# fractalclockwork/CS267_HW3

Hardware: NVIDIA B200
Metric: kmers_per_s_insert_plus_traverse (higher is better)
Workload: dtype u128

## Files before the change

### cs267_hw3_b200/csrc/capi.cu

```cuda
#include <algorithm>
#include <cmath>
#include <cstdio>
#include <cstdlib>
#include <cstring>
#include <string>
#include <vector>

#include <cub/device/device_radix_sort.cuh>

#include "../../include/kh_capi.h"
#include "kernels.cuh"
#include "ctable.cuh"

using namespace kh;

namespace {

struct DevBuf {
    void* p = nullptr;
    size_t cap = 0;
};

enum { EV_INS0, EV_INS1, EV_AS0, EV_WALK, EV_RANK, EV_AS1, EV_PACK0, EV_PACK1, EV_CLR0, EV_CLR1, EV_STAGE1, EV_BUILD0, EV_BUILD1, EV_COUNT };

// ... 1 lines not shown

struct kh_table {
    int k = 0, W = 1, device = 0, pl = 0, pb = 0, slot_bytes = 8, per_bucket = 4;
    int mlen = 0;
    int olen = 0;
    double lf = 0.5;
    u64 n_expected = 0, nbuckets = 0;
    cudaStream_t stream = nullptr, own_stream = nullptr, copy_stream = nullptr;
    void* table = nullptr;
    size_t table_bytes = 0;
    DevBuf starts;
    u64 n_starts = 0;
    DevBuf mask, tile_counts, tile_offs, scan_blocks;
    DevBuf part_cursor, grouped;
    DevBuf fine, chunk_cursor, overflow;
    int build_mode = 1;
    bool table_dirty = false;
    bool chunk_attr_set = false;
    int debug_cap_pct = 100;
    int partition_mode = -1;
    u64 part_bytes = 16ull << 20;
    bool part_attr_set = false;
    int ins_mode = 1;
    int warm_ahead = 1;
    Counters* d_ctr = nullptr;
    Counters* h_ctr = nullptr;
    DevBuf link, seglen, tmp, contig_len, contig_pre, contig_off, out;
    DevBuf stage[2], text_stage, scratch_a, scratch_b, scratch_c;
    DevBuf sort_keys[2], sort_vals[2], sort_tmp;
    void* h_out = nullptr; size_t h_out_cap = 0;
    void* h_off = nullptr; size_t h_off_cap = 0;
    u32 split_shift = 5, seg_chars = 64;
    cudaEvent_t ev[EV_COUNT] = {};
    cudaEvent_t ev_copied[2] = {}, ev_consumed[2] = {};
    cudaEvent_t ev_built = nullptr, ev_gathered = nullptr;
    bool have_ins = false, have_as = false, have_pack = false, have_clr = false, have_build = false, have_stage = false;
    u64 n_launches = 0;
    kh_stats stats = {};
    std::string err;
    int sm_count = 148, walk_blocks_per_sm = 0, rank_blocks_per_sm = 0;
    u64 last_contig_bytes = 0, last_n_contigs = 0;
    struct CtState {
        bool on = false, sealed = false, sharded = false, attr_set = false, connected = false;
        bool assembled = false;
        CtGeom g = {};
        CtCaps caps = {};
        CtPeers pe = {};
        u32 epoch = 0;
        u64 n_local_max = 0, n_total = 0, n_starts_max = 0, out_cap = 0;
        u64 n_starts_host = 0;
        DevBuf xin_vals, xin_chunk, xin_cnt, xin_done, xout_cursor, extra_vals, extra_chunk, extra_cnt, fine, chunk_cursor,
               chunk_base, pool_off, seg_base, ext_key, meta, pool, inbox, inbox_cnt, out_cursor, flags,
               answers, req_seg, g_link, g_meta, g_pool, g_hdr;
        bool slow = false;
        void* ipc_opened[kMaxRanks][24] = {};
    } ct;
    int ct_env = 1;
};

namespace {

int fail(kh_table* t, int status, const std::string& msg) {
    if (t) t->err = msg;
    return status;
}

#define KH_CUDA(t, expr)                                                                         \
    do {                                                                                         \
        cudaError_t e_ = (expr);                                                                 \
        if (e_ != cudaSuccess)                                                                   \
            return fail((t), e_ == cudaErrorMemoryAllocation ? KH_ERR_NOMEM : KH_ERR_CUDA,       \
                        std::string(#expr) + ": " + cudaGetErrorString(e_));                     \
    } while (0)

#define KH_TRY(expr)                  \
    do {                              \
        const int rc_ = (expr);       \
        if (rc_ != KH_OK) return rc_; \
    } while (0)

int ensure(kh_table* t, DevBuf& b, size_t bytes, bool keep = false) {
    if (bytes <= b.cap && b.p) return KH_OK;
    const size_t want = std::max<size_t>(256, bytes + bytes / 8);
    void* np = nullptr;
    KH_CUDA(t, cudaMalloc(&np, want));
    if (b.p) {
        if (keep && b.cap) KH_CUDA(t, cudaMemcpyAsync(np, b.p, b.cap, cudaMemcpyDeviceToDevice, t->stream));
        KH_CUDA(t, cudaStreamSynchronize(t->stream));
        KH_CUDA(t, cudaFree(b.p));
    }
    b.p = np;
    b.cap = want;
    return KH_OK;
}

int ensure_pinned(kh_table* t, void*& p, size_t& cap, size_t bytes) {
    if (bytes <= cap && p) return KH_OK;
    if (p) KH_CUDA(t, cudaFreeHost(p));
    p = nullptr; cap = 0;
    const size_t want = std::max<size_t>(4096, bytes + bytes / 8);
    KH_CUDA(t, cudaHostAlloc(&p, want, cudaHostAllocDefault));
    cap = want;
    return KH_OK;
}

int status_from_errors(kh_table* t, u32 e) {
// ... 378 lines not shown
    c.n_local_max = n_local_max; c.n_total = n_total; c.n_starts_max = n_starts_max; c.sharded = sharded;
    const u64 nb_alloc = (u64)((long double)n_exp / (long double)t->lf / per_bucket) + C + 64;
    if (!t->table || t->table_bytes < nb_alloc * 32) {
        if (t->table) { KH_CUDA(t, cudaStreamSynchronize(t->stream)); KH_CUDA(t, cudaFree(t->table)); t->table = nullptr; }
        KH_CUDA(t, cudaMalloc(&t->table, nb_alloc * 32));
        t->table_bytes = nb_alloc * 32;
    }
    t->nbuckets = nb_alloc;
    c.caps.nbuckets_alloc = nb_alloc;
    const double share = (double)std::max<u64>(n_local_max, 1) / (double)world;
    u64 xin_cap = world > 1 ? (u64)((share * 1.05 + 64.0 * std::sqrt(share + 1.0) + 4096.0) * t->debug_cap_pct / 100.0) : 8;
    xin_cap = std::max<u64>(8, (xin_cap + 7) & ~7ull);
    if (xin_cap >= 0xFFFFFFF0ull) return fail(t, KH_ERR_ARG, "receive buffer too large");
    c.caps.xin_cap = (u32)xin_cap;
    c.caps.extra_cap = (u32)std::min<u64>(0x7FFFFFF0ull, t->debug_cap_pct < 100 ? n_local_max * (u64)world + 65536 : n_exp / 16 + 65536);
    const u64 hcap = sharded ? std::min<u64>(std::max<u64>(n_starts_max, 1), n_local_max + 1) : 0;
    c.caps.hcap = (u32)hcap;
    const u64 seg_cap = hcap + n_exp + 64;
    if (seg_cap >= (u64)kLocalMask - 16 && sharded) return fail(t, KH_ERR_ARG, "too many segments per GPU for 28-bit local ids");
    c.caps.seg_cap = (u32)std::min<u64>(seg_cap, 0xFFFFFF00ull);
    c.caps.pool_cap = n_exp + 16 * C + 64;
    c.caps.inbox_cap = world > 1 ? (u32)std::min<u64>(0x7FFFFFF0ull, ((n_exp + n_local_max) / world) * 9 / 8 + 4096) : 1;
    c.out_cap = n_total + std::max<u64>(n_starts_max, 1) * (u64)(t->k + 1) + 64;
    KH_TRY(ensure(t, c.xin_vals, (u64)world * xin_cap * sizeof(V)));
    KH_TRY(ensure(t, c.xin_chunk, (u64)world * xin_cap * sizeof(u32)));
    KH_TRY(ensure(t, c.xin_cnt, kMaxRanks * sizeof(u32)));
    KH_TRY(ensure(t, c.xin_done, (kMaxRanks + 1) * sizeof(u32)));
    KH_TRY(ensure(t, c.xout_cursor, kMaxRanks * sizeof(u32)));
    KH_TRY(ensure(t, c.extra_vals, (u64)c.caps.extra_cap * sizeof(V)));
    KH_TRY(ensure(t, c.extra_chunk, (u64)c.caps.extra_cap * sizeof(u32)));
    KH_TRY(ensure(t, c.extra_cnt, 16));
    KH_TRY(ensure(t, c.fine, C * (u64)((slots_max + 15) & ~15u) * sizeof(V)));
    KH_TRY(ensure(t, c.chunk_cursor, (C + 1) * sizeof(u32)));
    KH_TRY(ensure(t, c.chunk_base, (C + 2) * sizeof(u32)));
    KH_TRY(ensure(t, c.pool_off, (C + 2) * sizeof(u32)));
    KH_TRY(ensure(t, c.seg_base, (C + 1) * sizeof(u32)));
    KH_TRY(ensure(t, c.pool, c.caps.pool_cap + 64));
    KH_TRY(ensure(t, c.inbox, (u64)world * c.caps.inbox_cap * sizeof(CtReq<W>)));
    KH_TRY(ensure(t, c.inbox_cnt, kMaxRanks * sizeof(u32)));
    KH_TRY(ensure(t, c.out_cursor, kMaxRanks * sizeof(u32)));
    KH_TRY(ensure(t, c.flags, 2 * kMaxRanks * sizeof(u32)));
    c.caps.g_seg_stride = world > 1 ? ((n_local_max + 1 + n_exp + 64 + 15) & ~15ull) : 0;
    c.caps.g_pool_stride = world > 1 ? ((c.caps.pool_cap + 64 + 15) & ~15ull) : 0;
    KH_TRY(ensure(t, c.answers, std::max<u64>(16, (u64)(world > 1 ? world : 0) * c.caps.inbox_cap * sizeof(u32))));
    KH_TRY(ensure(t, c.req_seg, std::max<u64>(16, (u64)(world > 1 ? world : 0) * c.caps.inbox_cap * sizeof(u32))));
    KH_TRY(ensure(t, c.g_link, std::max<u64>(16, (u64)world * c.caps.g_seg_stride * sizeof(u64))));
    KH_TRY(ensure(t, c.g_meta, std::max<u64>(16, (u64)world * c.caps.g_seg_stride * sizeof(u64))));
    KH_TRY(ensure(t, c.g_pool, std::max<u64>(16, (u64)world * c.caps.g_pool_stride)));
    KH_TRY(ensure(t, c.g_hdr, 2 * kMaxRanks * sizeof(u32)));
    if (sharded) {
        KH_TRY(ensure(t, t->link, seg_cap * sizeof(u64)));
        KH_TRY(ensure(t, c.meta, seg_cap * sizeof(u64)));
        KH_TRY(ensure(t, c.ext_key, seg_cap * sizeof(V)));
        KH_TRY(ensure(t, t->contig_len, (hcap + 2) * sizeof(u32)));
        KH_TRY(ensure(t, t->contig_pre, (hcap + 2) * sizeof(u32)));
        KH_TRY(ensure(t, t->contig_off, (hcap + 2) * sizeof(u64)));
        KH_TRY(ensure(t, t->out, c.out_cap));
        KH_TRY(ensure(t, t->starts, (hcap + 1) * sizeof(V)));
        const u64 ntiles = (n_local_max + kInsTile - 1) / kInsTile + 1;
        KH_TRY(ensure(t, t->mask, (ntiles + 1) * (kInsTile / 32) * sizeof(u32)));
        KH_TRY(ensure(t, t->tile_counts, (ntiles + 1) * sizeof(u32)));
        KH_TRY(ensure(t, t->tile_offs, (ntiles + 1) * sizeof(u64)));
        KH_TRY(ensure(t, t->scan_blocks, ((std::max(ntiles, hcap + 2) + kScanTile - 1) / kScanTile + 2) * sizeof(u64)));
    }
    KH_TRY(ct_reset_staging(t));
    KH_CUDA(t, cudaMemsetAsync(c.inbox_cnt.p, 0, kMaxRanks * sizeof(u32), t->stream));
    KH_CUDA(t, cudaMemsetAsync(c.flags.p, 0, 2 * kMaxRanks * sizeof(u32), t->stream));
    KH_CUDA(t, cudaStreamSynchronize(t->stream));
    if (!c.attr_set) {
        KH_CUDA(t, cudaFuncSetAttribute(ct_build_kernel<W>, cudaFuncAttributeMaxDynamicSharedMemorySize, (int)CtBuild<W>::kSmem));
        KH_CUDA(t, cudaFuncSetAttribute(ct_build_kernel<W>, cudaFuncAttributePreferredSharedMemoryCarveout, (int)cudaSharedmemCarveoutMaxShared));
        KH_CUDA(t, cudaFuncSetAttribute(ct_stage_kernel<W>, cudaFuncAttributeMaxDynamicSharedMemorySize, (int)ct_stage_smem(W, 8)));
        c.attr_set = true;
    }
    memset(&c.pe, 0, sizeof(c.pe));
    c.pe.world = world; c.pe.rank = rank;
    c.epoch = 0;
    ct_set_self(t);
    c.on = true; c.sealed = false;
    return KH_OK;
}

int ct_barrier(kh_table* t, int round = -1) {
    auto& c = t->ct;
    if (c.pe.world <= 1) return KH_OK;
    ++c.epoch;
    ct_barrier_kernel<<<1, 32, 0, t->stream>>>(c.pe, c.epoch & 0x7FFFFFFFu, t->d_ctr, round);
    ++t->n_launches;
    KH_CUDA(t, cudaGetLastError());
    return KH_OK;
}

template <int W>
int ct_stage(kh_table* t, const unsigned char* recs, u64 n) {
    typedef typename Slot<W>::value_t V;
    auto& c = t->ct;
    if (n == 0) return KH_OK;
    if (n >= 0xFFF00000ull) return fail(t, KH_ERR_ARG, "at most 2^32-2^20 records per insert call; split the batch");
    const u64 ntiles = (n + kInsTile - 1) / kInsTile;
    if (!c.sharded) {
        KH_TRY(ensure(t, t->mask, (ntiles + 1) * (kInsTile / 32) * sizeof(u32)));
        KH_TRY(ensure(t, t->tile_counts, (ntiles + 1) * sizeof(u32)));
        KH_TRY(ensure(t, t->tile_offs, (ntiles + 1) * sizeof(u64)));
        KH_TRY(ensure(t, t->scan_blocks, ((ntiles + kScanTile - 1) / kScanTile + 2) * sizeof(u64)));
        KH_TRY(ensure(t, t->starts, (c.n_starts_host + n + 1) * sizeof(V), true));
        c.caps.hcap = (u32)std::min<u64>(0xFFFFFF00ull, c.n_starts_host + n + 1);
// ... 7 lines not shown
    KH_TRY(device_scan(t, static_cast<u32*>(t->tile_counts.p), ntiles, static_cast<u64*>(t->tile_offs.p), &t->d_ctr->scan_total));
    ct_scatter_starts_kernel<W><<<(unsigned)((ntiles * 32 + 255) / 256), 256, 0, t->stream>>>(
        recs, n, t->k, static_cast<u32*>(t->mask.p), static_cast<u64*>(t->tile_offs.p), ntiles, static_cast<V*>(t->starts.p),
        t->d_ctr, c.caps.hcap);
    ct_bump_starts_kernel<<<1, 1, 0, t->stream>>>(t->d_ctr, c.caps.hcap);
    KH_CUDA(t, cudaGetLastError());
    t->n_launches += 3;
    KH_CUDA(t, cudaEventRecord(t->ev[EV_STAGE1], t->stream));
    t->have_stage = true;
    c.sealed = false; c.assembled = false;
    t->table_dirty = true;
    return KH_OK;
}

__global__ void ct_init_seal_kernel(Counters* c, u32 hcap) {
    c->next_seg = hcap;
    c->n_inserted = 0;
    c->n_duplicates = 0;
}
__global__ void ct_init_assemble_kernel(Counters* c) {
    c->n_nodes = 0;
    c->contig_bytes = 0;
    c->rank_rounds = 0;
    c->rank_done = 0;
    c->need_jump = 0;
    c->use_jump = 0;
    for (int i = 0; i < 40; ++i) c->flags[i] = 0;
}
__global__ void ct_reset_nodes_kernel(Counters* c) { c->n_nodes = 0; }

template <int W>
int ct_seal_publish(kh_table* t) {
    auto& c = t->ct;
    if (c.pe.world > 1) {
        ct_publish_xin_kernel<<<1, 32, 0, t->stream>>>(c.pe, c.caps, static_cast<const u32*>(c.xout_cursor.p));
        ++t->n_launches;
        KH_CUDA(t, cudaGetLastError());
    }
    return ct_barrier(t);
}
template <int W>
int ct_seal_build(kh_table* t) {
    typedef typename Slot<W>::value_t V;
    auto& c = t->ct;
    const u32 C = c.g.chunks_per_rank;
    if (!c.sharded) {
        const u64 hcap = c.n_starts_host + 1;
        const u64 seg_cap = hcap + std::max<u64>(t->n_expected, 1) + 64;
        if (seg_cap >= 0xFFFFFF00ull) return fail(t, KH_ERR_ARG, "too many segments for 32-bit ids");
        c.caps.hcap = (u32)hcap; c.caps.seg_cap = (u32)seg_cap;
        KH_TRY(ensure(t, t->link, seg_cap * sizeof(u64)));
        KH_TRY(ensure(t, c.meta, seg_cap * sizeof(u64)));
        KH_TRY(ensure(t, c.ext_key, seg_cap * sizeof(V)));
        ct_set_self(t);
    }
    ct_init_seal_kernel<<<1, 1, 0, t->stream>>>(t->d_ctr, c.caps.hcap);
    if (c.pe.world > 1) {
        u32* done = static_cast<u32*>(c.xin_done.p);
        ct_xin_scatter_kernel<W><<<(unsigned)t->sm_count * 8, 256, 0, t->stream>>>(
            static_cast<const V*>(c.xin_vals.p), static_cast<const u32*>(c.xin_chunk.p), static_cast<const u32*>(c.xin_cnt.p), done,
            c.g, c.caps, static_cast<u32*>(c.chunk_cursor.p), static_cast<V*>(c.fine.p), t->d_ctr);
        ct_extra_kernel<W><<<64, 256, 0, t->stream>>>(static_cast<const V*>(c.extra_vals.p), static_cast<const u32*>(c.extra_chunk.p),
                                                      static_cast<const u32*>(c.extra_cnt.p), done + kMaxRanks, c.caps, C,
                                                      static_cast<u32*>(c.chunk_cursor.p), static_cast<V*>(c.fine.p), t->d_ctr);
        ct_mark_filed_kernel<<<1, 32, 0, t->stream>>>(static_cast<const u32*>(c.xin_cnt.p), done, static_cast<const u32*>(c.extra_cnt.p),
                                                      done + kMaxRanks, c.caps, c.pe.world);
        t->n_launches += 3;
    }
    ct_layout_kernel<<<1, 1024, 0, t->stream>>>(static_cast<const u32*>(c.chunk_cursor.p), C, c.g, c.caps, (u32)Slot<W>::kPerBucket,
                                                CtBuild<W>::kMaxSlots, static_cast<u32*>(c.chunk_base.p), static_cast<u32*>(c.pool_off.p), t->d_ctr);
    t->n_launches += 2;
    KH_CUDA(t, cudaEventRecord(t->ev[EV_BUILD0], t->stream));
    ct_build_kernel<W><<<C, kCtBuildThreads, CtBuild<W>::kSmem, t->stream>>>(
        static_cast<const V*>(c.fine.p), static_cast<const u32*>(c.chunk_cursor.p), static_cast<const u32*>(c.chunk_base.p),
        static_cast<const u32*>(c.pool_off.p), static_cast<V*>(t->table), static_cast<u32*>(c.seg_base.p),
        static_cast<u64*>(t->link.p), static_cast<u64*>(c.meta.p), static_cast<V*>(c.ext_key.p),
        static_cast<unsigned char*>(c.pool.p), c.g, c.caps, t->d_ctr);
    KH_CUDA(t, cudaGetLastError());
    KH_CUDA(t, cudaEventRecord(t->ev[EV_BUILD1], t->stream));
    t->have_build = true;
    c.sealed = true;
    return KH_OK;
}

constexpr int kCtMaxRounds = 24;
constexpr int kCtParts = 8 + kCtMaxRounds;
constexpr u32 kCtWalkMaxSteps = 512;

template <int W>
int ct_assemble_part(kh_table* t, int part) {
    typedef typename Slot<W>::value_t V;
    auto& c = t->ct;
    const unsigned gb = (unsigned)t->sm_count * 8;
    u64* link = static_cast<u64*>(t->link.p);
    CtGathered gt = {};
    for (int r = 0; r < c.pe.world; ++r) {
        const bool me = r == c.pe.rank;
        gt.link[r] = me ? link : static_cast<const u64*>(c.g_link.p) + (u64)r * c.caps.g_seg_stride;
        gt.meta[r] = me ? static_cast<const u64*>(c.meta.p) : static_cast<const u64*>(c.g_meta.p) + (u64)r * c.caps.g_seg_stride;
        gt.pool[r] = me ? static_cast<const unsigned char*>(c.pool.p) : static_cast<const unsigned char*>(c.g_pool.p) + (u64)r * c.caps.g_pool_stride;
    }
    switch (part) {
    case 0:
        if (c.assembled) { c.sealed = false; c.assembled = false; }
        c.slow = false;
        KH_CUDA(t, cudaEventRecord(t->ev[EV_AS0], t->stream));
// ... 1 lines not shown
        return ct_barrier(t);
    case 1: {
        if (!c.sealed) { KH_TRY(ct_seal_build<W>(t)); KH_CUDA(t, cudaEventRecord(t->ev[EV_INS1], t->stream)); t->have_ins = true; }
        if (!c.sharded) {
            const u64 hc = c.n_starts_host;
            KH_TRY(ensure(t, t->contig_len, (hc + 3) * sizeof(u32)));
            KH_TRY(ensure(t, t->contig_pre, (hc + 3) * sizeof(u32)));
            KH_TRY(ensure(t, t->contig_off, (hc + 3) * sizeof(u64)));
            c.out_cap = t->h_ctr->n_inserted + c.n_starts_host * (u64)(t->k + 1) + 64;
            ct_set_self(t);
        }
        if (c.pe.world > 1) {
            KH_CUDA(t, cudaEventRecord(t->ev_built, t->stream));
            KH_CUDA(t, cudaStreamWaitEvent(t->copy_stream, t->ev_built, 0));
            ct_gather_kernel<<<gb, 256, 0, t->copy_stream>>>(c.pe, c.caps, link, static_cast<const u64*>(c.meta.p), static_cast<const unsigned char*>(c.pool.p),
                                                             static_cast<const u32*>(c.pool_off.p), c.g.chunks_per_rank, t->d_ctr, 0);
            KH_CUDA(t, cudaEventRecord(t->ev_gathered, t->copy_stream));
            ++t->n_launches;
        }
        ct_init_assemble_kernel<<<1, 1, 0, t->stream>>>(t->d_ctr);
        KH_CUDA(t, cudaMemsetAsync(c.out_cursor.p, 0, kMaxRanks * sizeof(u32), t->stream));
        ct_stub_kernel<W><<<std::max(1u, std::min(gb, (c.caps.hcap + 255u) / 256u)), 256, 0, t->stream>>>(
            static_cast<const V*>(t->starts.p), t->d_ctr, c.caps.hcap, link, static_cast<u64*>(c.meta.p), static_cast<V*>(c.ext_key.p));
        ct_resolve_kernel<W><<<gb, 256, 0, t->stream>>>(static_cast<const V*>(t->table), static_cast<const u32*>(c.chunk_base.p),
                                                        static_cast<const u32*>(c.seg_base.p), link, static_cast<const V*>(c.ext_key.p),
                                                        c.g, c.pe, c.caps, static_cast<u32*>(c.out_cursor.p), static_cast<u32*>(c.req_seg.p), t->d_ctr);
        if (c.pe.world > 1) { ct_publish_inbox_kernel<<<1, 32, 0, t->stream>>>(c.pe, c.caps, static_cast<const u32*>(c.out_cursor.p)); ++t->n_launches; }
        t->n_launches += 3;
        KH_CUDA(t, cudaGetLastError());
        return ct_barrier(t);
    }
    case 2:
        if (c.pe.world > 1) {
            ct_answer_kernel<W><<<gb, 256, 0, t->stream>>>(static_cast<const V*>(t->table), static_cast<const u32*>(c.chunk_base.p),
                                                           static_cast<const u32*>(c.seg_base.p), static_cast<const CtReq<W>*>(c.inbox.p),
                                                           static_cast<const u32*>(c.inbox_cnt.p), c.g, c.pe, c.caps);
            KH_CUDA(t, cudaGetLastError());
            ++t->n_launches;
        }
        return ct_barrier(t);
    case 3:
        if (c.pe.world > 1) {
            ct_apply_kernel<<<gb, 256, 0, t->stream>>>(link, static_cast<const u32*>(c.answers.p), static_cast<const u32*>(c.req_seg.p),
                                                       static_cast<const u32*>(c.out_cursor.p), c.caps, c.pe.world, c.pe.rank);
            ct_gather_kernel<<<gb, 256, 0, t->stream>>>(c.pe, c.caps, link, static_cast<const u64*>(c.meta.p), static_cast<const unsigned char*>(c.pool.p),
                                                        static_cast<const u32*>(c.pool_off.p), c.g.chunks_per_rank, t->d_ctr, 1);
            KH_CUDA(t, cudaStreamWaitEvent(t->stream, t->ev_gathered, 0));
            KH_CUDA(t, cudaGetLastError());
            t->n_launches += 2;
        }
        KH_CUDA(t, cudaEventRecord(t->ev[EV_WALK], t->stream));
        return ct_barrier(t);
    case 4:
        ct_walk_len_kernel<<<gb, 256, 0, t->stream>>>(gt, link, c.caps, t->k, kCtWalkMaxSteps, static_cast<u32*>(t->contig_len.p), t->d_ctr);
        KH_CUDA(t, cudaGetLastError());
        ++t->n_launches;
        return ct_barrier(t, -2);
    case 5: {
        KH_TRY(device_scan(t, static_cast<u32*>(t->contig_len.p), (u64)c.caps.hcap + 1, static_cast<u64*>(t->contig_off.p), &t->d_ctr->contig_bytes));
        KH_CUDA(t, cudaEventRecord(t->ev[EV_RANK], t->stream));
        ct_walk_emit_kernel<W><<<gb, 256, 0, t->stream>>>(gt, link, static_cast<const V*>(t->starts.p), c.caps, t->k, static_cast<const u32*>(t->contig_len.p),
                                                          static_cast<const u64*>(t->contig_off.p), c.out_cap, static_cast<char*>(t->out.p), t->d_ctr);
        KH_CUDA(t, cudaGetLastError());
        ++t->n_launches;
        KH_CUDA(t, cudaEventRecord(t->ev[EV_AS1], t->stream));
        t->have_as = true;
        return KH_OK;
    }
    case 6: {
        KH_TRY(read_counters(t));
        c.slow = (c.pe.world > 1 ? t->h_ctr->use_jump : t->h_ctr->need_jump) != 0;
        if (!c.slow) return KH_OK;
        c.assembled = true;
        ct_rank_round_kernel<<<gb, 256, 0, t->stream>>>(c.pe, link, c.caps, t->d_ctr, t->d_ctr->flags, 0);
        KH_CUDA(t, cudaGetLastError());
        ++t->n_launches;
        return ct_barrier(t, 0);
    }
    case 6 + kCtMaxRounds: {
        if (!c.slow) return KH_OK;
        ct_reset_nodes_kernel<<<1, 1, 0, t->stream>>>(t->d_ctr);
        ct_lengths_kernel<<<gb, 256, 0, t->stream>>>(c.pe, link, c.caps, t->k, static_cast<u32*>(t->contig_len.p),
                                                     static_cast<u32*>(t->contig_pre.p), t->d_ctr);
        ct_claim_kernel<<<gb, 256, 0, t->stream>>>(c.pe, link, c.caps, static_cast<const u32*>(t->contig_len.p), t->d_ctr);
        KH_CUDA(t, cudaGetLastError());
        t->n_launches += 3;
        KH_TRY(device_scan(t, static_cast<u32*>(t->contig_len.p), (u64)c.caps.hcap + 1, static_cast<u64*>(t->contig_off.p), &t->d_ctr->contig_bytes));
        KH_CUDA(t, cudaEventRecord(t->ev[EV_RANK], t->stream));
        return ct_barrier(t);
    }
    case 7 + kCtMaxRounds:
        if (!c.slow) return KH_OK;
        ct_emit_kernel<<<gb, 256, 0, t->stream>>>(c.pe, link, static_cast<const u64*>(c.meta.p), static_cast<const unsigned char*>(c.pool.p),
                                                  c.caps, t->d_ctr, t->k);
        ct_emit_heads_kernel<W><<<gb, 256, 0, t->stream>>>(static_cast<const V*>(t->starts.p), c.caps, t->k, static_cast<const u32*>(t->contig_len.p),
                                                          static_cast<const u64*>(t->contig_off.p), t->d_ctr, c.out_cap, static_cast<char*>(t->out.p));
        KH_CUDA(t, cudaGetLastError());
        t->n_launches += 2;
        KH_CUDA(t, cudaEventRecord(t->ev[EV_AS1], t->stream));
        t->have_as = true;
        return ct_barrier(t);
    default: {
        if (part < 7 || part >= 6 + kCtMaxRounds) return fail(t, KH_ERR_ARG, "unknown assemble part");
        if (!c.slow) return KH_OK;
        const int r = part - 6;
        ct_rank_round_kernel<<<gb, 256, 0, t->stream>>>(c.pe, link, c.caps, t->d_ctr, t->d_ctr->flags, r);
        KH_CUDA(t, cudaGetLastError());
        ++t->n_launches;
        return ct_barrier(t, r);
    }
    }
}

int ct_finish(kh_table* t, u32* bits_out) {
    auto& c = t->ct;
    KH_TRY(read_counters(t));
    const Counters& h = *t->h_ctr;
// ... 129 lines not shown
    ck(cudaStreamCreateWithFlags(&t->copy_stream, cudaStreamNonBlocking));
    t->stream = t->own_stream;
    if (!use_ct) ck(cudaMalloc(&t->table, t->table_bytes));
    ck(cudaMalloc((void**)&t->d_ctr, sizeof(Counters)));
    ck(cudaHostAlloc((void**)&t->h_ctr, sizeof(Counters), cudaHostAllocDefault));
    for (auto& e : t->ev) ck(cudaEventCreate(&e));
    for (auto& e : t->ev_copied) ck(cudaEventCreateWithFlags(&e, cudaEventDisableTiming));
    for (auto& e : t->ev_consumed) ck(cudaEventCreateWithFlags(&e, cudaEventDisableTiming));
    ck(cudaEventCreateWithFlags(&t->ev_built, cudaEventDisableTiming));
    ck(cudaEventCreateWithFlags(&t->ev_gathered, cudaEventDisableTiming));
    if (rc != KH_OK) { fprintf(stderr, "libkh_b200: kh_create: %s\n", t->err.c_str()); return bail(rc); }
    if (!use_ct) ck(cudaMemsetAsync(t->table, 0, t->table_bytes, t->stream));
    ck(cudaMemsetAsync(t->d_ctr, 0, sizeof(Counters), t->stream));
    ck(cudaStreamSynchronize(t->stream));
    if (rc != KH_OK) return bail(rc);
    memset(t->h_ctr, 0, sizeof(Counters));
    int v = env_int("KH_SPLIT_BUCKETS", 0);
    if (v > 0 && set_option(t, "split_buckets", v) != KH_OK) fprintf(stderr, "libkh_b200: ignoring KH_SPLIT_BUCKETS=%d\n", v);
    t->mlen = env_int("KH_LOCALITY", 0) ? minimizer_len(k) : 0;
    t->olen = env_int("KH_OWNER_LOCALITY", 1) ? owner_minimizer_len(k) : 0;
    if (env_int("KH_OWNER_MLEN", 0) > 0) t->olen = std::min(k, env_int("KH_OWNER_MLEN", 0));
    t->partition_mode = env_int("KH_PARTITION", -1);
    t->build_mode = env_int("KH_BUILD", t->W == 1 ? 1 : 0);
    t->debug_cap_pct = std::max(1, env_int("KH_DEBUG_CAP_PCT", 100));
    t->ins_mode = env_int("KH_INS_MODE", 1);
    t->warm_ahead = env_int("KH_WARM_AHEAD", 1);
    v = env_int("KH_PART_MB", 0);
    if (v > 0) t->part_bytes = (u64)v << 20;
    v = env_int("KH_SEG_CHARS", 0);
    if (v > 0 && set_option(t, "seg_chars", v) != KH_OK) fprintf(stderr, "libkh_b200: ignoring KH_SEG_CHARS=%d\n", v);
    if (use_ct) {
        rc = t->W == 1 ? ct_setup<1>(t, 0, 1, n_expected, n_expected, n_expected, false)
                       : ct_setup<2>(t, 0, 1, n_expected, n_expected, n_expected, false);
        if (rc != KH_OK) { fprintf(stderr, "libkh_b200: kh_create: %s\n", t->err.c_str()); return bail(rc); }
    }
    t->err.clear();
    *out = t;
    return KH_OK;
}

int kh_destroy(kh_table* t) {
    if (!t) return KH_OK;
    cudaSetDevice(t->device);
    if (t->own_stream) cudaStreamSynchronize(t->own_stream);
    DevBuf* bufs[] = {&t->starts, &t->mask, &t->tile_counts, &t->tile_offs, &t->scan_blocks, &t->link, &t->seglen,
                      &t->tmp, &t->part_cursor, &t->grouped, &t->fine, &t->chunk_cursor, &t->overflow, &t->contig_len, &t->contig_pre, &t->contig_off, &t->out, &t->stage[0], &t->stage[1],
                      &t->text_stage, &t->scratch_a, &t->scratch_b, &t->scratch_c, &t->sort_keys[0], &t->sort_keys[1], &t->sort_vals[0], &t->sort_vals[1], &t->sort_tmp};
    for (DevBuf* b : bufs) if (b->p) cudaFree(b->p);
    for (auto& row : t->ct.ipc_opened) for (void* q : row) if (q) cudaIpcCloseMemHandle(q);
    {
        auto& c = t->ct;
        for (DevBuf* b : {&c.xin_vals, &c.xin_chunk, &c.xin_cnt, &c.xin_done, &c.xout_cursor, &c.extra_vals, &c.extra_chunk, &c.extra_cnt, &c.fine,
                          &c.chunk_cursor, &c.chunk_base, &c.pool_off, &c.seg_base, &c.ext_key, &c.meta, &c.pool, &c.inbox, &c.inbox_cnt,
                          &c.out_cursor, &c.flags, &c.answers, &c.req_seg, &c.g_link, &c.g_meta, &c.g_pool, &c.g_hdr})
            if (b->p) cudaFree(b->p);
    }
    if (t->table) cudaFree(t->table);
    if (t->d_ctr) cudaFree(t->d_ctr);
    if (t->h_ctr) cudaFreeHost(t->h_ctr);
    if (t->h_out) cudaFreeHost(t->h_out);
    if (t->h_off) cudaFreeHost(t->h_off);
    for (auto& e : t->ev) if (e) cudaEventDestroy(e);
    for (auto& e : t->ev_copied) if (e) cudaEventDestroy(e);
    for (auto& e : t->ev_consumed) if (e) cudaEventDestroy(e);
    if (t->ev_built) cudaEventDestroy(t->ev_built);
    if (t->ev_gathered) cudaEventDestroy(t->ev_gathered);
    if (t->own_stream) cudaStreamDestroy(t->own_stream);
    if (t->copy_stream) cudaStreamDestroy(t->copy_stream);
    cudaGetLastError();
    delete t;
    return KH_OK;
}

int kh_clear(kh_table* t) {
    if (!t) return KH_ERR_ARG;
    KH_CUDA(t, cudaSetDevice(t->device));
    KH_CUDA(t, cudaEventRecord(t->ev[EV_CLR0], t->stream));
    if (t->ct.on) {
        KH_TRY(ct_reset_staging(t));
        t->ct.sealed = false; t->ct.assembled = false;
        t->ct.n_starts_host = 0;
    } else {
        KH_CUDA(t, cudaMemsetAsync(t->table, 0, t->table_bytes, t->stream));
    }
    KH_CUDA(t, cudaMemsetAsync(t->d_ctr, 0, sizeof(Counters), t->stream));
    KH_CUDA(t, cudaEventRecord(t->ev[EV_CLR1], t->stream));
    t->have_clr = true;
    t->table_dirty = false;
    t->n_starts = 0;
    memset(t->h_ctr, 0, sizeof(Counters));
    t->stats.n_contigs = t->stats.n_nodes = t->stats.contig_bytes = t->stats.n_segments = 0;
    t->stats.rank_rounds = 0;
    t->last_contig_bytes = t->last_n_contigs = 0;
    return KH_OK;
}

int kh_set_stream(kh_table* t, void* cuda_stream) {
    if (!t) return KH_ERR_ARG;
    KH_CUDA(t, cudaSetDevice(t->device));
    KH_CUDA(t, cudaStreamSynchronize(t->stream));
    t->stream = cuda_stream ? static_cast<cudaStream_t>(cuda_stream) : cudaStreamLegacy;
    return KH_OK;
}

int kh_sync(kh_table* t) {
    if (!t) return KH_ERR_ARG;
    KH_CUDA(t, cudaSetDevice(t->device));
// ... 440 lines not shown
int kh_shard_insert(kh_table* t, const void* pairs_dev, uint64_t n) {
    if (!t || (n && !pairs_dev)) return KH_ERR_ARG;
    KH_TRY(shard_require(t));
    KH_CUDA(t, cudaSetDevice(t->device));
    if (!t->have_ins || t->ct.sealed || !t->table_dirty) KH_CUDA(t, cudaEventRecord(t->ev[EV_INS0], t->stream));
    return t->W == 1 ? ct_stage<1>(t, static_cast<const unsigned char*>(pairs_dev), n)
                     : ct_stage<2>(t, static_cast<const unsigned char*>(pairs_dev), n);
}

int kh_shard_assemble_parts(void) { return kCtParts; }

int kh_shard_assemble_part(kh_table* t, int part) {
    if (!t) return KH_ERR_ARG;
    KH_TRY(shard_require(t));
    KH_CUDA(t, cudaSetDevice(t->device));
    return t->W == 1 ? ct_assemble_part<1>(t, part) : ct_assemble_part<2>(t, part);
}

int kh_shard_assemble(kh_table* t) {
    for (int part = 0; part < kCtParts; ++part) KH_TRY(kh_shard_assemble_part(t, part));
    return KH_OK;
}

int kh_shard_finish(kh_table* t, int* error_bits_out) {
    if (!t) return KH_ERR_ARG;
    KH_TRY(shard_require(t));
    KH_CUDA(t, cudaSetDevice(t->device));
    u32 bits = 0;
    KH_TRY(ct_finish(t, &bits));
    if (error_bits_out) *error_bits_out = (int)bits;
    return KH_OK;
}

int kh_shard_result(kh_table* t, const char** contigs_dev, const uint64_t** offsets_dev,
                    uint64_t* n_contigs, uint64_t* contig_bytes, uint64_t* n_nodes) {
    if (!t) return KH_ERR_ARG;
    KH_TRY(shard_require(t));
    if (contigs_dev) *contigs_dev = static_cast<const char*>(t->out.p);
    if (offsets_dev) *offsets_dev = static_cast<const uint64_t*>(t->contig_off.p);
    if (n_contigs) *n_contigs = t->stats.n_contigs;
    if (contig_bytes) *contig_bytes = t->stats.contig_bytes;
    if (n_nodes) *n_nodes = t->stats.n_nodes;
    return KH_OK;
}

int kh_debug_buffer(kh_table* t, const char* name, void** ptr_out, uint64_t* bytes_out) {
    if (!t || !name || !ptr_out || !bytes_out) return KH_ERR_ARG;
    auto& c = t->ct;
    const std::string n(name);
    const DevBuf* b = nullptr;
    if (n == "link") b = &t->link; else if (n == "meta") b = &c.meta; else if (n == "ext_key") b = &c.ext_key;
    else if (n == "chunk_base") b = &c.chunk_base; else if (n == "seg_base") b = &c.seg_base; else if (n == "chunk_cursor") b = &c.chunk_cursor;
    else if (n == "inbox_cnt") b = &c.inbox_cnt; else if (n == "out_cursor") b = &c.out_cursor; else if (n == "xin_cnt") b = &c.xin_cnt;
    else if (n == "contig_len") b = &t->contig_len; else if (n == "pool") b = &c.pool;
    else if (n == "counters") { *ptr_out = t->d_ctr; *bytes_out = sizeof(Counters); return KH_OK; }
    else if (n == "caps") {
        static thread_local uint64_t v[8];
        v[0] = c.caps.hcap; v[1] = c.caps.seg_cap; v[2] = c.caps.inbox_cap; v[3] = c.caps.xin_cap; v[4] = c.g.chunks_per_rank; v[5] = 0;
        v[6] = c.epoch; v[7] = 0;
        *ptr_out = v; *bytes_out = sizeof(v); return KH_OK;
    }
    if (!b) return fail(t, KH_ERR_ARG, "unknown buffer " + n);
    *ptr_out = b->p; *bytes_out = b->cap;
    return KH_OK;
}

uint64_t kh_slot_bytes(int k) { return (ct_supported(k) ? ct_slot_words(k) : ((2 * k + 6 <= 64) ? 1 : 2)) * 8; }

int kh_copy_to_host(kh_table* t, void* dst_host, const void* src_dev, uint64_t bytes) {
    if (!t || (bytes && (!dst_host || !src_dev))) return KH_ERR_ARG;
    KH_CUDA(t, cudaSetDevice(t->device));
    if (bytes) KH_CUDA(t, cudaMemcpyAsync(dst_host, src_dev, bytes, cudaMemcpyDeviceToHost, t->stream));
    KH_CUDA(t, cudaStreamSynchronize(t->stream));
    return KH_OK;
}
int kh_copy_device(kh_table* t, void* dst_dev, const void* src_dev, uint64_t bytes) {
    if (!t || (bytes && (!dst_dev || !src_dev))) return KH_ERR_ARG;
    KH_CUDA(t, cudaSetDevice(t->device));
    if (bytes) KH_CUDA(t, cudaMemcpyAsync(dst_dev, src_dev, bytes, cudaMemcpyDefault, t->stream));
    return KH_OK;
}
int kh_device_alloc(void** ptr, uint64_t bytes) {
    if (!ptr) return KH_ERR_ARG;
    if (cudaMalloc(ptr, bytes ? bytes : 1) != cudaSuccess) { cudaGetLastError(); *ptr = nullptr; return KH_ERR_NOMEM; }
    return KH_OK;
}
int kh_device_alloc_on(int device, void** ptr, uint64_t bytes) {
    if (!ptr) return KH_ERR_ARG;
    if (cudaSetDevice(device) != cudaSuccess) { cudaGetLastError(); *ptr = nullptr; return KH_ERR_CUDA; }
    return kh_device_alloc(ptr, bytes);
}
int kh_device_free(void* ptr) {
    if (ptr && cudaFree(ptr) != cudaSuccess) { cudaGetLastError(); return KH_ERR_CUDA; }
    return KH_OK;
}

}
```

### cs267_hw3_b200/csrc/ctable.cuh

```cuda
#pragma once
#include "kernels.cuh"

namespace kh {

#ifndef KH_CT_BUCKETS2
#define KH_CT_BUCKETS2 2176
#endif
#ifndef KH_CT_THREADS
#define KH_CT_THREADS 512
#endif
#ifndef KH_CT_MINBLOCKS
#define KH_CT_MINBLOCKS 2
#endif
#ifndef KH_CT_JUMPS
#define KH_CT_JUMPS 3
#endif
template <int W> struct CtBuild {
    static constexpr u32 kMaxBuckets = (W == 1) ? 1536u : (u32)KH_CT_BUCKETS2;
    static constexpr u32 kMaxSlots = kMaxBuckets * (u32)Slot<W>::kPerBucket;
    static constexpr u32 kOffSucc = kMaxBuckets * 32u;
    static constexpr u32 kOffPd = kOffSucc + kMaxSlots * 2u;
    static constexpr u32 kOffOff = kOffPd + kMaxSlots * 4u;
    static constexpr u32 kOffCode = kOffOff + kMaxSlots * 2u;
    static constexpr u32 kSmem = kOffCode + kMaxSlots;
// ... 827 lines not shown
        if (src == g.rank) continue;
        const u32 n = min(inbox_cnt[src], caps.inbox_cap);
        const CtReq<W>* __restrict__ box = inbox + (u64)src * caps.inbox_cap;
        for (u32 i = blockIdx.x * blockDim.x + threadIdx.x; i < n; i += gridDim.x * blockDim.x) {
            const CtReq<W> e = box[i];
            pe.answers[src][(u64)g.rank * caps.inbox_cap + i] = ct_resolve_one<W>(table, chunk_base, seg_base, e.chunk, e.key, my_bits);
        }
    }
}

__global__ void __launch_bounds__(256)
ct_apply_kernel(u64* __restrict__ link, const u32* __restrict__ answers, const u32* __restrict__ req_seg, const u32* __restrict__ out_cursor,
                const CtCaps caps, int world, int rank) {
    for (int o = 0; o < world; ++o) {
        if (o == rank) continue;
        const u32 n = min(out_cursor[o], caps.inbox_cap);
        const u64 base = (u64)o * caps.inbox_cap;
        for (u32 i = blockIdx.x * blockDim.x + threadIdx.x; i < n; i += gridDim.x * blockDim.x)
            reinterpret_cast<u32*>(link + req_seg[base + i])[1] = answers[base + i];
    }
}

__global__ void __launch_bounds__(256)
ct_gather_kernel(const CtPeers pe, const CtCaps caps, const u64* __restrict__ link, const u64* __restrict__ meta,
                 const unsigned char* __restrict__ pool, const u32* __restrict__ pool_off, u32 nchunks, const Counters* __restrict__ ctr,
                 int what) {
    const u32 nseg = min(ctr->next_seg, caps.seg_cap);
    const u32 first = caps.hcap;
    const u32 cnt = nseg > first ? nseg - first : 0u;
    const u64 pool_vecs = ((u64)pool_off[nchunks] + 15u) >> 4;
    const u64 tid = (u64)blockIdx.x * blockDim.x + threadIdx.x, stride = (u64)gridDim.x * blockDim.x;
    for (int d = 1; d < pe.world; ++d) {
        const int p = (pe.rank + d) % pe.world;
        u64* gl = pe.g_link[p] + (u64)pe.rank * caps.g_seg_stride;
        u64* gm = pe.g_meta[p] + (u64)pe.rank * caps.g_seg_stride;
        uint4* gp = reinterpret_cast<uint4*>(pe.g_pool[p] + (u64)pe.rank * caps.g_pool_stride);
        if (what == 1) {
            for (u64 i = tid; i < cnt; i += stride) gl[first + i] = link[first + i];
        } else {
            for (u64 i = tid; i < cnt; i += stride) gm[first + i] = meta[first + i];
            const uint4* sp = reinterpret_cast<const uint4*>(pool);
            for (u64 i = tid; i < pool_vecs; i += stride) gp[i] = sp[i];
            if (tid == 0) { pe.g_hdr[p][2 * pe.rank] = nseg; pe.g_hdr[p][2 * pe.rank + 1] = (u32)pool_vecs; }
        }
    }
}

struct CtGathered {
    const u64* link[kMaxRanks];
    const u64* meta[kMaxRanks];
    const unsigned char* pool[kMaxRanks];
};

__global__ void __launch_bounds__(256)
ct_walk_len_kernel(const CtGathered gt, const u64* __restrict__ link, const CtCaps caps, int k, u32 max_steps,
                   u32* __restrict__ contig_len, Counters* ctr) {
    const u32 n_starts = (u32)min(ctr->n_starts_dev, (u64)caps.hcap);
    u64 nodes = 0;
    u32 err = 0, too_long = 0;
    for (u64 c = (u64)blockIdx.x * blockDim.x + threadIdx.x; c <= caps.hcap; c += (u64)gridDim.x * blockDim.x) {
        if (c >= n_starts) { contig_len[c] = 0; continue; }
        u32 gid = (u32)(__ldg(link + c) >> 32), chars = 0, e = 0, steps = 0;
        if (gid == kLinkMissing) e = kErrNotFound;
        else if (gid == kLinkConverge) e = kErrConverge;
        else if (gid >= kLinkCtFirstMarker) e = kErrInternal;
        while (!e) {
            const u64 l = __ldg(gt.link[gid >> kRankShift] + (gid & kLocalMask));
            const u32 hi = (u32)(l >> 32);
            if (hi == kLinkTail) { chars += (u32)(__ldg(gt.meta[gid >> kRankShift] + (gid & kLocalMask)) & 0xFFFFFFu); break; }
            if (hi == kLinkMissing) { e = kErrNotFound; break; }
            if (hi == kLinkConverge) { e = kErrConverge; break; }
            if (hi >= kLinkCtFirstMarker) { e = kErrInternal; break; }
            chars += (u32)l;
            gid = hi;
            if (++steps > max_steps) { too_long = 1; break; }
        }
        if (e || too_long) { err |= e; contig_len[c] = 0; continue; }
        contig_len[c] = (u32)k + chars + 1u;
        nodes += (u64)chars + 1u;
    }
    nodes = warp_sum_u64(nodes);
    err = __reduce_or_sync(kFullMask, err);
    too_long = __reduce_or_sync(kFullMask, too_long);
    if (lane_id() == 0) {
        if (nodes) atomicAdd(&ctr->n_nodes, nodes);
        if (err) atomicOr(&ctr->errors, err);
        if (err & kErrInternal) atomicOr(&ctr->err_where, kSiteStubOpen);
        if (too_long) atomicOr(&ctr->need_jump, 1u);
    }
}

__device__ __forceinline__ void ct_copy_chars(char* dst, const unsigned char* src, u32 n) {
    while (n && (reinterpret_cast<uintptr_t>(dst) & 3u)) { *dst++ = (char)*src++; --n; }
    if (n >= 4) {
        const u32 sh = ((u32)reinterpret_cast<uintptr_t>(src) & 3u) * 8u;
        const u32* sw = reinterpret_cast<const u32*>(reinterpret_cast<uintptr_t>(src) & ~(uintptr_t)3);
        u32 w0 = __ldg(sw);
        u32* dw = reinterpret_cast<u32*>(dst);
        const u32 nw = n >> 2;
        for (u32 i = 0; i < nw; ++i) {
            const u32 w1 = __ldg(sw + i + 1);
            dw[i] = __funnelshift_r(w0, w1, sh);
            w0 = w1;
        }
        dst += 4 * nw; src += 4 * nw; n &= 3u;
    }
    while (n) { *dst++ = (char)*src++; --n; }
}

template <int W>
__global__ void __launch_bounds__(256)
ct_walk_emit_kernel(const CtGathered gt, const u64* __restrict__ link, const typename Slot<W>::value_t* __restrict__ starts,
                    const CtCaps caps, int k, const u32* __restrict__ contig_len, const u64* __restrict__ contig_off, u64 out_cap,
                    char* __restrict__ out, const Counters* __restrict__ ctr) {
    typedef Slot<W> S;
    if (ctr->use_jump || ctr->need_jump || (ctr->errors & (kErrConverge | kErrCycle | kErrInternal | kErrNotFound)) || ctr->contig_bytes > out_cap) return;
    const u32 n_starts = (u32)min(ctr->n_starts_dev, (u64)caps.hcap);
    for (u64 c = (u64)blockIdx.x * blockDim.x + threadIdx.x; c < n_starts; c += (u64)gridDim.x * blockDim.x) {
        const u32 len = contig_len[c];
        if (len == 0) continue;
        char* dst = out + contig_off[c];
        char* const end = dst + len - 1u;
        *end = '\n';
        {
            const typename S::value_t v0 = starts[c];
            int j = 0;
            while (j < k && (reinterpret_cast<uintptr_t>(dst) & 3u)) { *dst++ = (char)ext_char(S::base_at(v0, k, j)); ++j; }
            for (; j + 4 <= k; j += 4, dst += 4) {
                const u32 w = (u32)ext_char(S::base_at(v0, k, j)) | ((u32)ext_char(S::base_at(v0, k, j + 1)) << 8) |
                              ((u32)ext_char(S::base_at(v0, k, j + 2)) << 16) | ((u32)ext_char(S::base_at(v0, k, j + 3)) << 24);
                *reinterpret_cast<u32*>(dst) = w;
            }
            for (; j < k; ++j) *dst++ = (char)ext_char(S::base_at(v0, k, j));
        }
        u32 gid = (u32)(__ldg(link + c) >> 32);
        for (;;) {
            const u32 r = gid >> kRankShift, i = gid & kLocalMask;
            const u64 l = __ldg(gt.link[r] + i), mt = __ldg(gt.meta[r] + i);
            const u32 n = (u32)(mt & 0xFFFFFFu);
            if (dst + n > end) break;
            ct_copy_chars(dst, gt.pool[r] + (mt >> 24), n);
            dst += n;
            const u32 hi = (u32)(l >> 32);
            if (hi >= kLinkCtFirstMarker) break;
            gid = hi;
        }
    }
}

__device__ __forceinline__ u64* ct_peer_link(const CtPeers& pe, u32 gid) { return pe.link[gid >> kRankShift] + (gid & kLocalMask); }
__device__ __forceinline__ bool ct_is_end_marker(u32 hi) { return hi == kLinkTail || hi == kLinkClaimed || hi == kLinkMissing || hi == kLinkConverge; }

__global__ void __launch_bounds__(256)
ct_rank_round_kernel(const CtPeers pe, u64* __restrict__ link, const CtCaps caps, Counters* ctr, u32* __restrict__ moved, int round) {
    if (ctr->rank_done || (round > 0 && moved[round - 1] == 0)) return;
    const u32 nseg = min(ctr->next_seg, caps.seg_cap);
    bool any = false;
    for (u64 i = (u64)blockIdx.x * blockDim.x + threadIdx.x; i < nseg; i += (u64)gridDim.x * blockDim.x) {
        const u64 li = __ldcg(link + i);
        const u32 pi = (u32)(li >> 32), si = (u32)li;
        if (pi >= kLinkCtFirstMarker) continue;
        if (si & kLinkFinalBit) continue;
        const u64 lp = __ldcg(ct_peer_link(pe, pi));
        const u32 pp = (u32)(lp >> 32), sp = (u32)lp;
        if (ct_is_end_marker(pp)) { __stcg(link + i, li | kLinkFinalBit); continue; }
        if (pp >= kLinkCtFirstMarker) continue;
        __stcg(link + i, ((u64)pp << 32) | (u32)((si + (sp & kLinkDistMask)) | (sp & kLinkFinalBit)));
        any = true;
    }
    if (__any_sync(kFullMask, any) && lane_id() == 0) moved[round] = 1;
}

__global__ void __launch_bounds__(256)
ct_lengths_kernel(const CtPeers pe, const u64* __restrict__ link, const CtCaps caps, int k,
                  u32* __restrict__ contig_len, u32* __restrict__ contig_pre, Counters* ctr) {
    const u32 n_starts = (u32)min(ctr->n_starts_dev, (u64)caps.hcap);
    u64 nodes = 0;
    u32 err = 0;
    for (u64 c = (u64)blockIdx.x * blockDim.x + threadIdx.x; c <= caps.hcap; c += (u64)gridDim.x * blockDim.x) {
        if (c >= n_starts) { contig_len[c] = 0; continue; }
        const u64 lc = __ldcg(link + c);
        const u32 pc = (u32)(lc >> 32);
        u32 e = 0, tail_hi = 0, chars = 0, pre = 0;
        if (pc == kLinkMissing) e = kErrNotFound;
        else if (pc == kLinkConverge) e = kErrConverge;
        else if (pc >= kLinkCtFirstMarker) { e = kErrInternal; atomicOr(&ctr->err_where, kSiteStubOpen); }
        else if (!((u32)lc & kLinkFinalBit)) e = kErrCycle;
        else {
            tail_hi = (u32)(__ldcg(ct_peer_link(pe, pc)) >> 32);
            if (tail_hi == kLinkMissing) e = kErrNotFound;
            else if (tail_hi == kLinkConverge) e = kErrConverge;
            else {
                pre = (u32)lc & kLinkDistMask;
                chars = pre + (u32)(pe.meta[pc >> kRankShift][pc & kLocalMask] & 0xFFFFFFu);
            }
        }
        if (e) { err |= e; contig_pre[c] = 0; contig_len[c] = 0; continue; }
        contig_pre[c] = pre;
// ... 126 lines not shown
```

Baseline: 12.68 billion.

## Emit contigs per segment in parallel using precomputed segment destinations

After: 12.98 billion (median of 6 runs). 2.4% higher.

```diff
diff --git a/cs267_hw3_b200/csrc/capi.cu b/cs267_hw3_b200/csrc/capi.cu
--- a/cs267_hw3_b200/csrc/capi.cu
+++ b/cs267_hw3_b200/csrc/capi.cu
@@ -77,6 +77,7 @@
         DevBuf xin_vals, xin_chunk, xin_cnt, xin_done, xout_cursor, extra_vals, extra_chunk, extra_cnt, fine, chunk_cursor,
                chunk_base, pool_off, seg_base, ext_key, meta, pool, inbox, inbox_cnt, out_cursor, flags,
                answers, req_seg, g_link, g_meta, g_pool, g_hdr;
+        DevBuf seg_dst;
         bool slow = false;
         void* ipc_opened[kMaxRanks][24] = {};
     } ct;
@@ -561,6 +562,7 @@
         KH_TRY(ensure(t, t->link, seg_cap * sizeof(u64)));
         KH_TRY(ensure(t, c.meta, seg_cap * sizeof(u64)));
         KH_TRY(ensure(t, c.ext_key, seg_cap * sizeof(V)));
+        KH_TRY(ensure(t, c.seg_dst, std::max<u64>(seg_cap, (u64)world * c.caps.g_seg_stride) * sizeof(u64)));
         KH_TRY(ensure(t, t->contig_len, (hcap + 2) * sizeof(u32)));
         KH_TRY(ensure(t, t->contig_pre, (hcap + 2) * sizeof(u32)));
         KH_TRY(ensure(t, t->contig_off, (hcap + 2) * sizeof(u64)));
@@ -674,6 +676,7 @@
         KH_TRY(ensure(t, t->link, seg_cap * sizeof(u64)));
         KH_TRY(ensure(t, c.meta, seg_cap * sizeof(u64)));
         KH_TRY(ensure(t, c.ext_key, seg_cap * sizeof(V)));
+        KH_TRY(ensure(t, c.seg_dst, seg_cap * sizeof(u64)));
         ct_set_self(t);
     }
     ct_init_seal_kernel<<<1, 1, 0, t->stream>>>(t->d_ctr, c.caps.hcap);
@@ -781,17 +784,23 @@
         KH_CUDA(t, cudaEventRecord(t->ev[EV_WALK], t->stream));
         return ct_barrier(t);
     case 4:
-        ct_walk_len_kernel<<<gb, 256, 0, t->stream>>>(gt, link, c.caps, t->k, kCtWalkMaxSteps, static_cast<u32*>(t->contig_len.p), t->d_ctr);
+        ct_seg_dst_clear_kernel<<<gb, 256, 0, t->stream>>>(static_cast<u64*>(c.seg_dst.p), static_cast<const u32*>(c.g_hdr.p), c.pe.world,
+                                                           c.pe.rank, c.caps, t->d_ctr);
+        ct_walk_len_kernel<<<gb, 256, 0, t->stream>>>(gt, link, c.caps, t->k, kCtWalkMaxSteps, static_cast<u32*>(t->contig_len.p),
+                                                      static_cast<u64*>(c.seg_dst.p), t->d_ctr);
         KH_CUDA(t, cudaGetLastError());
-        ++t->n_launches;
+        t->n_launches += 2;
         return ct_barrier(t, -2);
     case 5: {
         KH_TRY(device_scan(t, static_cast<u32*>(t->contig_len.p), (u64)c.caps.hcap + 1, static_cast<u64*>(t->contig_off.p), &t->d_ctr->contig_bytes));
         KH_CUDA(t, cudaEventRecord(t->ev[EV_RANK], t->stream));
-        ct_walk_emit_kernel<W><<<gb, 256, 0, t->stream>>>(gt, link, static_cast<const V*>(t->starts.p), c.caps, t->k, static_cast<const u32*>(t->contig_len.p),
-                                                          static_cast<const u64*>(t->contig_off.p), c.out_cap, static_cast<char*>(t->out.p), t->d_ctr);
+        ct_walk_heads_kernel<W><<<gb, 256, 0, t->stream>>>(static_cast<const V*>(t->starts.p), c.caps, t->k, static_cast<const u32*>(t->contig_len.p),
+                                                           static_cast<const u64*>(t->contig_off.p), c.out_cap, static_cast<char*>(t->out.p), t->d_ctr);
+        ct_walk_segs_kernel<<<gb, 256, 0, t->stream>>>(gt, static_cast<const u64*>(c.seg_dst.p), static_cast<const u32*>(c.g_hdr.p), c.pe.world,
+                                                       c.pe.rank, c.caps, t->k, static_cast<const u64*>(t->contig_off.p), c.out_cap,
+                                                       static_cast<char*>(t->out.p), t->d_ctr);
         KH_CUDA(t, cudaGetLastError());
-        ++t->n_launches;
+        t->n_launches += 2;
         KH_CUDA(t, cudaEventRecord(t->ev[EV_AS1], t->stream));
         t->have_as = true;
         return KH_OK;
@@ -1027,7 +1036,7 @@
         auto& c = t->ct;
         for (DevBuf* b : {&c.xin_vals, &c.xin_chunk, &c.xin_cnt, &c.xin_done, &c.xout_cursor, &c.extra_vals, &c.extra_chunk, &c.extra_cnt, &c.fine,
                           &c.chunk_cursor, &c.chunk_base, &c.pool_off, &c.seg_base, &c.ext_key, &c.meta, &c.pool, &c.inbox, &c.inbox_cnt,
-                          &c.out_cursor, &c.flags, &c.answers, &c.req_seg, &c.g_link, &c.g_meta, &c.g_pool, &c.g_hdr})
+                          &c.out_cursor, &c.flags, &c.answers, &c.req_seg, &c.g_link, &c.g_meta, &c.g_pool, &c.g_hdr, &c.seg_dst})
             if (b->p) cudaFree(b->p);
     }
     if (t->table) cudaFree(t->table);
@@ -1574,7 +1583,7 @@
     if (n == "link") b = &t->link; else if (n == "meta") b = &c.meta; else if (n == "ext_key") b = &c.ext_key;
     else if (n == "chunk_base") b = &c.chunk_base; else if (n == "seg_base") b = &c.seg_base; else if (n == "chunk_cursor") b = &c.chunk_cursor;
     else if (n == "inbox_cnt") b = &c.inbox_cnt; else if (n == "out_cursor") b = &c.out_cursor; else if (n == "xin_cnt") b = &c.xin_cnt;
-    else if (n == "contig_len") b = &t->contig_len; else if (n == "pool") b = &c.pool;
+    else if (n == "contig_len") b = &t->contig_len; else if (n == "pool") b = &c.pool; else if (n == "seg_dst") b = &c.seg_dst;
     else if (n == "counters") { *ptr_out = t->d_ctr; *bytes_out = sizeof(Counters); return KH_OK; }
     else if (n == "caps") {
         static thread_local uint64_t v[8];
diff --git a/cs267_hw3_b200/csrc/ctable.cuh b/cs267_hw3_b200/csrc/ctable.cuh
--- a/cs267_hw3_b200/csrc/ctable.cuh
+++ b/cs267_hw3_b200/csrc/ctable.cuh
@@ -903,9 +903,26 @@
     const unsigned char* pool[kMaxRanks];
 };
 
+constexpr u64 kSegDstNone = ~0ull;
+
+__device__ __forceinline__ u32 ct_gathered_nseg(int r, int rank, const u32* __restrict__ g_hdr, const CtCaps& caps,
+                                                const Counters* __restrict__ ctr) {
+    return r == rank ? min(ctr->next_seg, caps.seg_cap) : (u32)min((u64)g_hdr[2 * r], caps.g_seg_stride);
+}
+
+__global__ void __launch_bounds__(256)
+ct_seg_dst_clear_kernel(u64* __restrict__ seg_dst, const u32* __restrict__ g_hdr, int world, int rank, const CtCaps caps,
+                        const Counters* __restrict__ ctr) {
+    for (int r = 0; r < world; ++r) {
+        const u32 nseg = ct_gathered_nseg(r, rank, g_hdr, caps, ctr);
+        u64* d = seg_dst + (u64)r * caps.g_seg_stride;
+        for (u64 i = (u64)caps.hcap + (u64)blockIdx.x * blockDim.x + threadIdx.x; i < nseg; i += (u64)gridDim.x * blockDim.x) d[i] = kSegDstNone;
+    }
+}
+
 __global__ void __launch_bounds__(256)
 ct_walk_len_kernel(const CtGathered gt, const u64* __restrict__ link, const CtCaps caps, int k, u32 max_steps,
-                   u32* __restrict__ contig_len, Counters* ctr) {
+                   u32* __restrict__ contig_len, u64* __restrict__ seg_dst, Counters* ctr) {
     const u32 n_starts = (u32)min(ctr->n_starts_dev, (u64)caps.hcap);
     u64 nodes = 0;
     u32 err = 0, too_long = 0;
@@ -917,8 +934,15 @@
         else if (gid >= kLinkCtFirstMarker) e = kErrInternal;
         while (!e) {
             const u64 l = __ldg(gt.link[gid >> kRankShift] + (gid & kLocalMask));
+            u64* const dst = seg_dst + (u64)(gid >> kRankShift) * caps.g_seg_stride + (gid & kLocalMask);
             const u32 hi = (u32)(l >> 32);
-            if (hi == kLinkTail) { chars += (u32)(__ldg(gt.meta[gid >> kRankShift] + (gid & kLocalMask)) & 0xFFFFFFu); break; }
+            if (hi == kLinkTail) {
+                const u32 n = (u32)(__ldg(gt.meta[gid >> kRankShift] + (gid & kLocalMask)) & 0xFFFFFFu);
+                if (atomicExch(reinterpret_cast<unsigned long long*>(dst), (unsigned long long)((c << 32) | chars)) != kSegDstNone) { too_long = 1; break; }
+                chars += n;
+                break;
+            }
+            *dst = (c << 32) | chars;
             if (hi == kLinkMissing) { e = kErrNotFound; break; }
             if (hi == kLinkConverge) { e = kErrConverge; break; }
             if (hi >= kLinkCtFirstMarker) { e = kErrInternal; break; }
@@ -941,60 +965,93 @@
     }
 }
 
-__device__ __forceinline__ void ct_copy_chars(char* dst, const unsigned char* src, u32 n) {
-    while (n && (reinterpret_cast<uintptr_t>(dst) & 3u)) { *dst++ = (char)*src++; --n; }
-    if (n >= 4) {
-        const u32 sh = ((u32)reinterpret_cast<uintptr_t>(src) & 3u) * 8u;
-        const u32* sw = reinterpret_cast<const u32*>(reinterpret_cast<uintptr_t>(src) & ~(uintptr_t)3);
-        u32 w0 = __ldg(sw);
-        u32* dw = reinterpret_cast<u32*>(dst);
-        const u32 nw = n >> 2;
-        for (u32 i = 0; i < nw; ++i) {
-            const u32 w1 = __ldg(sw + i + 1);
-            dw[i] = __funnelshift_r(w0, w1, sh);
-            w0 = w1;
-        }
-        dst += 4 * nw; src += 4 * nw; n &= 3u;
-    }
-    while (n) { *dst++ = (char)*src++; --n; }
-}
-
-template <int W>
-__global__ void __launch_bounds__(256)
-ct_walk_emit_kernel(const CtGathered gt, const u64* __restrict__ link, const typename Slot<W>::value_t* __restrict__ starts,
-                    const CtCaps caps, int k, const u32* __restrict__ contig_len, const u64* __restrict__ contig_off, u64 out_cap,
-                    char* __restrict__ out, const Counters* __restrict__ ctr) {
+__device__ __forceinline__ bool ct_walk_emit_skipped(const Counters* __restrict__ ctr, u64 out_cap) {
+    return ctr->use_jump || ctr->need_jump || (ctr->errors & (kErrConverge | kErrCycle | kErrInternal | kErrNotFound)) || ctr->contig_bytes > out_cap;
+}
+
+__device__ __forceinline__ u64 ct_shfl(u64 v, int src) { return __shfl_sync(kFullMask, v, src); }
+__device__ __forceinline__ u128 ct_shfl(u128 v, int src) { return u128{__shfl_sync(kFullMask, v.lo, src), __shfl_sync(kFullMask, v.hi, src)}; }
+
+template <int W>
+__global__ void __launch_bounds__(256)
+ct_walk_heads_kernel(const typename Slot<W>::value_t* __restrict__ starts, const CtCaps caps, int k, const u32* __restrict__ contig_len,
+                     const u64* __restrict__ contig_off, u64 out_cap, char* __restrict__ out, const Counters* __restrict__ ctr) {
     typedef Slot<W> S;
-    if (ctr->use_jump || ctr->need_jump || (ctr->errors & (kErrConverge | kErrCycle | kErrInternal | kErrNotFound)) || ctr->contig_bytes > out_cap) return;
+    if (ct_walk_emit_skipped(ctr, out_cap)) return;
     const u32 n_starts = (u32)min(ctr->n_starts_dev, (u64)caps.hcap);
-    for (u64 c = (u64)blockIdx.x * blockDim.x + threadIdx.x; c < n_starts; c += (u64)gridDim.x * blockDim.x) {
-        const u32 len = contig_len[c];
-        if (len == 0) continue;
-        char* dst = out + contig_off[c];
-        char* const end = dst + len - 1u;
-        *end = '\n';
-        {
-            const typename S::value_t v0 = starts[c];
-            int j = 0;
-            while (j < k && (reinterpret_cast<uintptr_t>(dst) & 3u)) { *dst++ = (char)ext_char(S::base_at(v0, k, j)); ++j; }
-            for (; j + 4 <= k; j += 4, dst += 4) {
-                const u32 w = (u32)ext_char(S::base_at(v0, k, j)) | ((u32)ext_char(S::base_at(v0, k, j + 1)) << 8) |
-                              ((u32)ext_char(S::base_at(v0, k, j + 2)) << 16) | ((u32)ext_char(S::base_at(v0, k, j + 3)) << 24);
-                *reinterpret_cast<u32*>(dst) = w;
-            }
-            for (; j < k; ++j) *dst++ = (char)ext_char(S::base_at(v0, k, j));
-        }
-        u32 gid = (u32)(__ldg(link + c) >> 32);
-        for (;;) {
-            const u32 r = gid >> kRankShift, i = gid & kLocalMask;
-            const u64 l = __ldg(gt.link[r] + i), mt = __ldg(gt.meta[r] + i);
-            const u32 n = (u32)(mt & 0xFFFFFFu);
-            if (dst + n > end) break;
-            ct_copy_chars(dst, gt.pool[r] + (mt >> 24), n);
-            dst += n;
-            const u32 hi = (u32)(l >> 32);
-            if (hi >= kLinkCtFirstMarker) break;
-            gid = hi;
+    const u32 lane = lane_id();
+    const u64 warp = ((u64)blockIdx.x * blockDim.x + threadIdx.x) >> 5, nwarps = ((u64)gridDim.x * blockDim.x) >> 5;
+    for (u64 c0 = warp * 32u; c0 < n_starts; c0 += nwarps * 32u) {
+        const u64 c = c0 + lane;
+        u32 len = 0;
+        u64 off = 0;
+        typename S::value_t v = {};
+        if (c < n_starts) { len = contig_len[c]; off = contig_off[c]; v = starts[c]; }
+        for (int q = 0; q < 32; ++q) {
+            const u32 lq = __shfl_sync(kFullMask, len, q);
+            const u64 oq = ct_shfl(off, q);
+            const typename S::value_t vq = ct_shfl(v, q);
+            if (lq == 0) continue;
+            for (u32 j = lane; j <= (u32)k; j += 32u)
+                out[oq + (j < (u32)k ? j : lq - 1u)] = j < (u32)k ? (char)ext_char(S::base_at(vq, k, (int)j)) : '\n';
+        }
+    }
+}
+
+__global__ void __launch_bounds__(256)
+ct_walk_segs_kernel(const CtGathered gt, const u64* __restrict__ seg_dst, const u32* __restrict__ g_hdr, int world, int rank,
+                    const CtCaps caps, int k, const u64* __restrict__ contig_off, u64 out_cap, char* __restrict__ out,
+                    const Counters* __restrict__ ctr) {
+    if (ct_walk_emit_skipped(ctr, out_cap)) return;
+    const u32 n_starts = (u32)min(ctr->n_starts_dev, (u64)caps.hcap);
+    const u32 lane = lane_id();
+    const u64 warp = ((u64)blockIdx.x * blockDim.x + threadIdx.x) >> 5, nwarps = ((u64)gridDim.x * blockDim.x) >> 5;
+    for (int r = 0; r < world; ++r) {
+        const u32 nseg = ct_gathered_nseg(r, rank, g_hdr, caps, ctr);
+        const u64* __restrict__ dsts = seg_dst + (u64)r * caps.g_seg_stride;
+        const u64* __restrict__ meta = gt.meta[r];
+        const unsigned char* __restrict__ pool = gt.pool[r];
+        for (u64 s0 = (u64)caps.hcap + warp * 32u; s0 < nseg; s0 += nwarps * 32u) {
+            const u64 s = s0 + lane;
+            u32 n = 0;
+            u64 dst = 0, src = 0;
+            if (s < nseg) {
+                const u64 d = dsts[s], mt = __ldg(meta + s);
+                const u32 c = (u32)(d >> 32);
+                if (c < n_starts) {
+                    dst = contig_off[c] + (u64)k + (u32)d;
+                    src = mt >> 24;
+                    n = (u32)(mt & 0xFFFFFFu);
+                    if (dst + n > contig_off[c + 1] - 1u) n = 0;
+                }
+            }
+            u32 pre = n;
+#pragma unroll
+            for (u32 o = 1; o < 32; o <<= 1) {
+                const u32 y = __shfl_up_sync(kFullMask, pre, o);
+                if (lane >= o) pre += y;
+            }
+            const u32 total = __shfl_sync(kFullMask, pre, 31);
+            pre -= n;
+            dst -= pre; src -= pre;
+            for (u32 b = 0; b < total; b += 128u) {
+                unsigned char ch[4];
+                u64 at[4];
+#pragma unroll
+                for (int q = 0; q < 4; ++q) {
+                    const u32 j = b + 32u * q + lane;
+                    u32 i = 0;
+#pragma unroll
+                    for (u32 h = 16; h; h >>= 1)
+                        if (__shfl_sync(kFullMask, pre, i + h) <= j) i += h;
+                    at[q] = __shfl_sync(kFullMask, dst, i) + j;
+                    const u64 sj = __shfl_sync(kFullMask, src, i) + j;
+                    ch[q] = j < total ? pool[sj] : 0;
+                }
+#pragma unroll
+                for (int q = 0; q < 4; ++q)
+                    if (b + 32u * q + lane < total) out[at[q]] = (char)ch[q];
+            }
         }
     }
 }
```
